# dwave-examples/image-generation

Hardware: AMD Instinct MI355X
Metric: DVAE+GRBM train-step images/s (MNIST) at 1/2/4/8 MI355X; loss parity vs CPU (higher is better)
Workload: dtype f32

## Files before the change

image-generation_amd/csrc/conv_plan.cpp:

```cpp
#include "conv_plan.h"

#include <algorithm>

namespace dvg {

PlanOptions plan_options() {
  PlanOptions o;
  o.precision = conv_precision_mode(); o.launch_mode = conv_launch_mode(0, 0);
  for (int i = 0; i < OPT_COUNT; ++i) o.v[i] = opt((Opt)i);
  return o;
}

namespace {
bool wino_mode_ok(const PlanOptions& o, ConvPass pass) { return pass == PASS_WGRAD || o.precision != 1; }

constexpr int WINO_MIN_BLOCKS = 512;

bool enc_wino_wanted(const PlanOptions& o, int64_t M, int Cout, ConvPass pass, bool training) {
  if (o.v[OPT_ENC_WINO] == 0 || !wino_mode_ok(o, pass)) return false;
  if (o.v[OPT_ENC_WINO] >= 1) return true;
  return conv_wino_blocks(M, Cout) >= (training ? WINO_MIN_BLOCKS : 256);
}

bool wino4_bit(const PlanOptions& o, int64_t mask, int bit) { return o.v[OPT_ENC_WINO4] != 0 && ((mask >> bit) & 1); }

bool wino4_block64(const PlanOptions& o, int l, bool dgrad, int64_t M, int Cin, int Cout, int L, int cus) {
  if (!wino4_bit(o, o.v[OPT_ENC_WINO4_MASK], enc_wino4_block64_bit(l, dgrad)) || !conv_wino4_block64_shape(M, Cin, Cout, L)) return false;
  return (int64_t)conv_wino4_stats_blocks(M) * (Cout / 64) >= 2 * (int64_t)(cus > 0 && cus < 256 ? cus : 256);
}

bool is_wino(ConvForm f) { return f == CF_WINO2 || f == CF_WINO4; }
WeightMap map9(const ConvLayer& y, bool dgrad) {
  const int mode = y.convt ? (dgrad ? WM_CONVT_DGRAD : WM_CONVT_FWD) : (dgrad ? WM_CONV_DGRAD : WM_CONV_FWD);
  return dgrad ? WeightMap{mode, y.Cout, y.Cin, 9} : WeightMap{mode, y.Cin, y.Cout, 9};
}
}

bool plan_enc_wino_fwd(int64_t M, int Cin, int Cout, int L, bool training, const PlanOptions& o) {
  return conv_wino_shape(M, Cin, Cout, L) && enc_wino_wanted(o, M, Cout, PASS_FWD, training);
}

int plan_enc_wino_cus(const PlanOptions& o, ConvPass pass, bool training) {
  if (pass == PASS_FWD) return (training && o.v[OPT_WINO_DYNAMIC] == 0) ? 192 : 0;
  if (pass == PASS_DGRAD) return o.v[OPT_ENC_DGRAD_CUS] > 0 ? (int)o.v[OPT_ENC_DGRAD_CUS] : WINO_CUS_ENC_DGRAD;
  return (int)o.v[OPT_ENC_WGRAD_CUS];
}

void plan_encoder_layers(int64_t B, int n, bool training, const PlanOptions& o, ConvLayer y[4]) {
  const int ch[5] = {1, 32, 64, 128, n};
  for (int l = 1; l < 4; ++l) {
    ConvLayer& c = y[l];
    c.M = B * (1024 >> (2 * l)); c.Cin = ch[l]; c.Cout = ch[l + 1]; c.L = 5 - l; c.ups = false; c.convt = false;
    c.form[PASS_FWD] = c.form[PASS_DGRAD] = c.form[PASS_WGRAD] = CF_DIRECT;
    c.block64[PASS_FWD] = c.block64[PASS_DGRAD] = false;
    if (plan_enc_wino_fwd(c.M, c.Cin, c.Cout, c.L, training, o))
      c.form[PASS_FWD] = wino4_bit(o, o.v[OPT_ENC_WINO4_MASK], l - 1) && conv_wino4_shape(c.M, c.Cin, c.Cout, c.L) ? CF_WINO4 : CF_WINO2;
    c.block64[PASS_FWD] = c.form[PASS_FWD] == CF_WINO4 &&
                          wino4_block64(o, l, false, c.M, c.Cin, c.Cout, c.L, plan_enc_wino_cus(o, PASS_FWD, training));
    if (!training) continue;
    if (conv_wino_shape(c.M, c.Cout, c.Cin, c.L) && enc_wino_wanted(o, c.M, c.Cin, PASS_DGRAD, true))
      c.form[PASS_DGRAD] = wino4_bit(o, o.v[OPT_ENC_WINO4_MASK], 2 + l) && conv_wino4_shape(c.M, c.Cout, c.Cin, c.L) ? CF_WINO4 : CF_WINO2;
    c.block64[PASS_DGRAD] = c.form[PASS_DGRAD] == CF_WINO4 &&
                            wino4_block64(o, l, true, c.M, c.Cout, c.Cin, c.L, plan_enc_wino_cus(o, PASS_DGRAD, true));
    if (conv_wino_wgrad_shape(c.M, c.Cin, c.Cout, c.L) && enc_wino_wanted(o, c.M, c.Cout, PASS_WGRAD, true) &&
        (o.v[OPT_ENC_WINO] >= 1 || conv_wino_shape(c.M, c.Cin, c.Cout, c.L)))
      c.form[PASS_WGRAD] = wino4_bit(o, o.v[OPT_ENC_WINO4_MASK], 5 + l) && conv_wino4_wgrad_shape(c.M, c.Cin, c.Cout, c.L) ? CF_WINO4 : CF_WINO2;
  }
}

void plan_decoder_layers(int64_t N, int n, const PlanOptions& o, ConvLayer y[3]) {
  const int ch[4] = {n, 128, 64, 32};
  for (int l = 0; l < 3; ++l) {
    ConvLayer& c = y[l];
    c.M = N * ((int64_t)4 << (2 * l)); c.Cin = ch[l]; c.Cout = ch[l + 1]; c.L = l + 1; c.ups = l > 0; c.convt = true;
    c.block64[PASS_FWD] = c.block64[PASS_DGRAD] = false;
    ConvForm base = CF_DIRECT;
    if (l == 0 && o.v[OPT_DEC_D22] != 0)
      base = o.v[OPT_DEC_LC0] != 0 && (o.v[OPT_DEC_LC0] > 0 || N >= 4096 || N * (int64_t)n >= (1 << 20)) && conv_pack_is_f32_kmajor(o.launch_mode) ? CF_LC0 : CF_D22;
    if (c.ups && o.v[OPT_DEC_FOLD] != 0 && conv_fold_ok(c.M / 4)) base = CF_FOLD;
    c.form[PASS_FWD] = c.form[PASS_DGRAD] = c.form[PASS_WGRAD] = base;
    if (!c.ups || o.v[OPT_DEC_WINO] == 0 || (o.v[OPT_DEC_WINO] < 0 && N < 8192)) continue;
// ... 109 lines not shown
```

image-generation_amd/csrc/conv_wino_wgrad.hip:

```cpp
#include <atomic>
#include <type_traits>

#include "conv_wino_common.h"

namespace dvg {

struct WinoWgradArgs {
  const float* in;
  const float* dy;
  float* slabs;
  int64_t M;
  int Cin, Cout, L;
  int isplit;
};

template <int WA, int WB>
struct WinoWgrad8Cfg {
  static constexpr int WK = 4 / (WA * WB);
  static constexpr int CIB = 32 * WA, COB = 32 * WB;
  static constexpr int QC = WK == 1 ? 8 : 4;
  static constexpr int NQ = QC * WK;
  static constexpr int V_B = NQ * CIB * 64, Z_B = NQ * COB * 64, STAGE = V_B + Z_B;
  static constexpr int LDS_BYTES = 2 * STAGE;
  static constexpr int NV = NQ * CIB / 2, NZ = NQ * COB / 2;
// ... 211 lines not shown
        for (int i = 0; i < NM; ++i) {
          if (i % MPG == 0) __builtin_amdgcn_sched_group_barrier(0x100, 2, 0);
          __builtin_amdgcn_sched_group_barrier(0x008, 1, 0);
          if (VPM > 0) __builtin_amdgcn_sched_group_barrier(0x002, VPM, 0);
          if (NST > 0 && ((i + 1) * NST) / NM - (i * NST) / NM >= 1) __builtin_amdgcn_sched_group_barrier(0x200, 1, 0);
          if (NST > 0 && ((i + 1) * NST) / NM - (i * NST) / NM >= 2) __builtin_amdgcn_sched_group_barrier(0x200, 1, 0);
          if (NST > 0 && ((i + 1) * NST) / NM - (i * NST) / NM >= 3) __builtin_amdgcn_sched_group_barrier(0x200, 1, 0);
        }
      }
      __builtin_amdgcn_sched_barrier(0);
#pragma unroll
      for (int e = NH; e < NGRP; ++e) {
        const int g = G0 + e * GSTEP;
        if (e + 1 < NGRP) load_grp(g + GSTEP, na, nb);
#pragma unroll
        for (int m = 0; m < 4; ++m)
          if (!UPS || m != 2)
            acc[4 * (g & 1) + m] = __builtin_amdgcn_mfma_f32_32x32x2f32(ca[m], cb[m], acc[4 * (g & 1) + m], 0, 0, 0);
        ca = na; cb = nb;
        __builtin_amdgcn_sched_group_barrier(0x100, 2, 0);
        __builtin_amdgcn_sched_group_barrier(0x008, MPG, 0);
      }
      __builtin_amdgcn_sched_barrier(0);
      __syncthreads();
    };
    for (int ch = 0; ch < nchunks; ch += 2) {
      chunk(ch, std::integral_constant<int, 0>{});
      chunk(ch + 1, std::integral_constant<int, 1>{});
    }
  };
  using R0 = std::integral_constant<int, 0>;
  using R1 = std::integral_constant<int, 1>;
  using R2 = std::integral_constant<int, 2>;
  using PX = std::integral_constant<int, -1>;
  if constexpr (UPS) {
    if (ps == 0) { if (is_v) run(R0{}, R0{}); else if (is_z) run(R1{}, R0{}); else run(R2{}, R0{}); }
    else { if (is_v) run(R0{}, R1{}); else if (is_z) run(R1{}, R1{}); else run(R2{}, R1{}); }
  } else {
    if (is_v) run(R0{}, PX{}); else if (is_z) run(R1{}, PX{}); else run(R2{}, PX{});
  }

  const size_t slab = ((size_t)blockIdx.z * C::WK + kg) * 16 * (size_t)a.Cin * a.Cout;
#pragma unroll
  for (int j = 0; j < 8; ++j) {
    if (UPS && (j & 3) == 2) continue;
    const int p = 8 * ps + j;
    if (UPS && (p >> 2) == 2) continue;
    float* dst = a.slabs + slab + ((size_t)p * a.Cin + a0 + wa * 32) * a.Cout + b0 + wb * 32 + c;
#pragma unroll
    for (int r = 0; r < 16; ++r) dst[(size_t)crow16(r, hh) * a.Cout] = acc[j][r];
  }
}

__global__ __launch_bounds__(256) void wino_wgrad_slabsum_kernel(float* __restrict__ slabs, int nslabs, int64_t pairs, int positions, int ups) {
  const int64_t total = positions * pairs;
  const int sub = threadIdx.x & 7;
  for (int64_t e = ((int64_t)blockIdx.x * 256 + threadIdx.x) >> 3; e < total; e += ((int64_t)gridDim.x * 256) >> 3) {
    if (ups) {
      const int p = (int)(e / pairs);
      if ((p >> 2) == 2 || (p & 3) == 2) continue;
    }
    float s = 0.f;
    for (int k0 = sub; k0 < nslabs; k0 += 64) {
      float v[8];
#pragma unroll
      for (int u = 0; u < 8; ++u) v[u] = k0 + 8 * u < nslabs ? slabs[(size_t)(k0 + 8 * u) * total + e] : 0.f;
#pragma unroll
      for (int u = 0; u < 8; ++u) if (k0 + 8 * u < nslabs) s += v[u];
    }
    s += __shfl_xor(s, 1, 64);
    s += __shfl_xor(s, 2, 64);
    s += __shfl_xor(s, 4, 64);
    if (sub == 0) slabs[e] = s;
  }
}

int launch_wino_wgrad_slabsum(float* slabs, int nslabs, int64_t pairs, int positions, int ups, hipStream_t s) {
  int64_t blocks = (positions * pairs * 8 + 255) / 256;
  if (blocks > 4096) blocks = 4096;
  DVG_LAUNCH(K_WGRAD_REDUCE, wino_wgrad_slabsum_kernel, dim3((unsigned)blocks), dim3(256), 0, s, slabs, nslabs, pairs, positions, ups);
  return DVG_OK;
}

__global__ __launch_bounds__(256) void wino_wgrad_reduce_kernel(const float* __restrict__ du, WeightMap map, float* __restrict__ grad_w, int ups) {
  const int64_t pairs = (int64_t)map.Ca * map.Cb;
  for (int64_t e = (int64_t)blockIdx.x * 256 + threadIdx.x; e < pairs; e += (int64_t)gridDim.x * 256) {
    float u[16];
#pragma unroll
    for (int p = 0; p < 16; ++p) u[p] = (ups && ((p >> 2) == 2 || (p & 3) == 2)) ? 0.f : du[(size_t)p * pairs + e];
    float t[3][4];
#pragma unroll
    for (int nu = 0; nu < 4; ++nu) {
      t[0][nu] = u[0 * 4 + nu] + 0.5f * (u[1 * 4 + nu] + u[2 * 4 + nu]);
      t[1][nu] = 0.5f * (u[1 * 4 + nu] - u[2 * 4 + nu]);
      t[2][nu] = 0.5f * (u[1 * 4 + nu] + u[2 * 4 + nu]) + u[3 * 4 + nu];
    }
    const int b = (int)(e % map.Cb), av = (int)(e / map.Cb);
#pragma unroll
    for (int r = 0; r < 3; ++r) {
      const float g0 = t[r][0] + 0.5f * (t[r][1] + t[r][2]);
      const float g1 = 0.5f * (t[r][1] - t[r][2]);
      const float g2 = 0.5f * (t[r][1] + t[r][2]) + t[r][3];
      grad_w[torch_weight_offset(map, 3 * r + 0, av, b)] = g0;
      grad_w[torch_weight_offset(map, 3 * r + 1, av, b)] = g1;
      grad_w[torch_weight_offset(map, 3 * r + 2, av, b)] = g2;
    }
  }
}

static bool wino_wgrad_shape_ok(int64_t M, int Cin, int Cout, int L) {
  if (L < 1 || L > 5 || M <= 0 || (M & (((int64_t)1 << (2 * L)) - 1))) return false;
  const bool t22 = Cin % 64 == 0 && Cout % 64 == 0, t12 = Cin == 32 && Cout % 64 == 0, t21 = Cin % 64 == 0 && Cout == 32;
  if (!(t22 || t12 || t21)) return false;
  if (M * (int64_t)(Cin > Cout ? Cin : Cout) * 4 >= 2147483647LL) return false;
  return true;
}
bool conv_wino_wgrad_shape(int64_t M, int Cin, int Cout, int L) { return wino_wgrad_shape_ok(M, Cin, Cout, L); }

struct WinoWgradGeom { int tiles, pgn, isplit, wk, nslabs; };
static WinoWgradGeom wino_wgrad_geom(int64_t M, int Cin, int Cout, int L, int cus) {
  WinoWgradGeom g;
  const bool full = Cin % 64 == 0 && Cout % 64 == 0;
  const int cib = Cin % 64 == 0 ? 64 : 32, cob = Cout % 64 == 0 ? 64 : 32, nq = 8;
  g.wk = full ? 1 : 2;
  g.tiles = (Cin / cib) * (Cout / cob);
  const int qi = 1 << (2 * L - 2);
  g.pgn = qi >= nq ? qi / nq : 1;
  const int ipc = qi >= nq ? 1 : nq / qi;
  const int n_img = (int)(M >> (2 * L));
  const int ichunks = (n_img + ipc - 1) / ipc;
  g.isplit = wino_slab_split(ichunks, g.tiles * g.pgn, cus).want;
  g.nslabs = g.pgn * g.isplit * g.wk;
  return g;
// ... 47 lines not shown
```

image-generation_amd/csrc/dev_hooks.cpp:

```cpp
#include "conv_plan.h"
#include "gibbs_plan.h"
#include "mmd_plan.h"
#include "../../include/dvg_dev.h"
using namespace dvg;

extern "C" int dvg_dev_conv_igemm(const float* in, const float* w, int mode, float* wp, const float* bias, float* out,
                                  float* stats, int64_t M, int Cin, int Cout, int L, int ntaps, int ups, int poolsum,
                                  int repack, float* splitk_ws, dvg_stream_t stream) {
  DVG_REQUIRE(in && w && wp && out, "dev_conv_igemm: null argument");
  hipStream_t s = (hipStream_t)stream;
  if (repack) DVG_TRY(launch_weight_pack(w, WeightMap{mode, Cin, Cout, ntaps}, wp, s, conv_launch_mode(M, Cout)));
  ConvArgs a;
  a.in = in; a.wp = wp; a.bias = bias; a.out = out; a.stats = stats;
  a.M = M; a.Cin = Cin; a.Cout = Cout; a.L = L; a.ntaps = ntaps; a.ups = ups; a.poolsum = poolsum;
  a.splitk_ws = splitk_ws;
  a.spin_a = opt(OPT_DEV_SPIN_OPERAND) != 0;
  return launch_conv_igemm(a, s);
}

extern "C" int dvg_dev_conv_wino(const float* in, const float* w, int mode, float* u, const float* bias, float* out,
                                 float* stats, int64_t M, int Cin, int Cout, int L, dvg_stream_t stream) {
  DVG_REQUIRE(in && w && u && out, "dev_conv_wino: null argument");
  hipStream_t s = (hipStream_t)stream;
  DVG_TRY(launch_wino_weight_pack(w, WeightMap{mode, Cin, Cout, 9}, u, s));
  ConvArgs a;
  a.in = in; a.wp = u; a.bias = bias; a.out = out; a.stats = stats;
  a.M = M; a.Cin = Cin; a.Cout = Cout; a.L = L; a.ntaps = 9; a.ups = 0; a.poolsum = 0;
  a.splitk_ws = nullptr;
  return launch_conv_wino(a, s);
}
extern "C" int dvg_dev_conv_wino4(const float* in, const float* w, int mode, float* u, const float* bias, float* out,
                                  float* stats, int64_t M, int Cin, int Cout, int L, int cus, int um, dvg_stream_t stream) {
  DVG_REQUIRE(in && w && u && out, "dev_conv_wino4: null argument");
  hipStream_t s = (hipStream_t)stream;
  DVG_TRY(launch_wino4_weight_pack(w, WeightMap{mode, Cin, Cout, 9}, u, s, um != 0));
  ConvArgs a;
  a.in = in; a.wp = u; a.bias = bias; a.out = out; a.stats = stats;
  a.M = M; a.Cin = Cin; a.Cout = Cout; a.L = L; a.ntaps = 9; a.ups = 0; a.poolsum = 0;
  a.splitk_ws = nullptr; a.wino_cus = cus; a.wino_um = um;
  const int64_t mask = opt(OPT_ENC_WINO4_MASK);
  a.wino4_block64 = um == 0 && L >= 2 && L <= 4 && ((mask >> enc_wino4_block64_bit(5 - L, mode != 0)) & 1) && conv_wino4_block64_shape(M, Cin, Cout, L);
  return launch_conv_wino4(a, s);
}
extern "C" int dvg_dev_conv_wino4_shape(int64_t M, int Cin, int Cout, int L) { return conv_wino4_shape(M, Cin, Cout, L) ? 1 : 0; }
extern "C" int dvg_dev_conv_wino_ok(int64_t M, int Cin, int Cout, int L) { return plan_enc_wino_fwd(M, Cin, Cout, L, true, plan_options()) ? 1 : 0; }

extern "C" int dvg_dev_plan_forms(int network, int64_t rows, int n_latents, int training, int out[15]) {
  DVG_REQUIRE(out && (network == 0 || network == 1) && rows >= 1 && n_latents >= 32 && n_latents % 32 == 0, "dev_plan_forms: bad argument");
  const PlanOptions o = plan_options();
  ConvLayer y[4];
  if (network == 0) plan_encoder_layers(rows, n_latents, training != 0, o, y);
  else plan_decoder_layers(rows, n_latents, o, y);
  for (int l = 0; l < 4; ++l)
// ... 26 lines not shown
  const int64_t v[19] = {p.form, p.lpc, p.waves, p.mb, p.nr, p.maxs, p.ch, p.fix, p.slots.n, p.chains_per_block, p.grid, p.threads,
                         (int64_t)p.lds, g.lane_has, g.lane_lpc, g.lane_mb, g.lane_nr, g.lane_rows, g.n_batches};
  for (int i = 0; i < 19; ++i) out[i] = v[i];
  return DVG_OK;
}
extern "C" int dvg_dev_gibbs_exchange_plan(int n, int n_colours, const int32_t* class_ptr, const int32_t* adj_ptr, int n_ladders,
                                           int n_replicas, int64_t out[20]) {
  DVG_REQUIRE(out && class_ptr && adj_ptr && n > 0 && n_colours > 0 && n_colours <= 64 && n_ladders > 0 && n_replicas >= 2 &&
                  n_replicas <= GIBBS_MAX_REPLICAS && (int64_t)n_ladders * n_replicas <= 0x7fffffff,
              "dev_gibbs_exchange_plan: bad argument");
  const GibbsGraphShape g = gibbs_graph_shape(n, n_colours, class_ptr, adj_ptr);
  GibbsDrawPlan p;
  int per_block = 0;
  DVG_TRY(gibbs_exchange_plan(g, n_ladders, n_replicas, opt(OPT_GIBBS_GENERIC), &p, &per_block));
  const int64_t v[20] = {p.form, p.lpc, p.waves, p.mb, p.nr, p.maxs, p.ch, p.fix, p.slots.n, p.chains_per_block, p.grid, p.threads,
                         (int64_t)p.lds, g.lane_has, g.lane_lpc, g.lane_mb, g.lane_nr, g.lane_rows, g.n_batches, per_block};
  for (int i = 0; i < 20; ++i) out[i] = v[i];
  return DVG_OK;
}
extern "C" int dvg_dev_conv_wino_stats_blocks(int64_t M, int Cout) { return conv_wino_stats_blocks(M, Cout); }

extern "C" size_t dvg_dev_conv_splitk_floats(int64_t M, int Cin, int Cout, int ntaps, int poolsum) {
  return conv_splitk_floats(M, Cin, Cout, ntaps, poolsum);
}

extern "C" int dvg_dev_conv_stats_blocks(int64_t M, int Cout) { return conv_stats_blocks(M, Cout); }

extern "C" size_t dvg_dev_wgrad_slab_floats(int64_t M, int Cin, int Cout, int ntaps) {
  return (size_t)wgrad_ksplit(M, Cin, Cout, ntaps) * ntaps * Cin * Cout;
}

extern "C" int dvg_dev_conv_wgrad(const float* in, const float* dy, float* slabs, float* grad_w, int mode, int64_t M,
                                  int Cin, int Cout, int L, int ntaps, int ups, dvg_stream_t stream) {
  DVG_REQUIRE(in && dy && slabs && grad_w, "dev_conv_wgrad: null argument");
  hipStream_t s = (hipStream_t)stream;
  WgradArgs wa;
  wa.in = in; wa.dy = dy; wa.slabs = slabs; wa.M = M; wa.Cin = Cin; wa.Cout = Cout; wa.L = L; wa.ntaps = ntaps;
  wa.ups = ups; wa.ksplit = wgrad_ksplit(M, Cin, Cout, ntaps);
  wa.spin_x = opt(OPT_DEV_SPIN_OPERAND) != 0;
  DVG_TRY(launch_conv_wgrad(wa, s));
  return launch_wgrad_reduce(slabs, wa.ksplit, WeightMap{mode, Cin, Cout, ntaps}, grad_w, s);
}

extern "C" size_t dvg_dev_wino_wgrad_slab_floats(int64_t M, int Cin, int Cout, int L) {
  return conv_wino_wgrad_shape(M, Cin, Cout, L) ? conv_wino_wgrad_slab_floats(M, Cin, Cout, L) : 0;
}

extern "C" int dvg_dev_conv_wino_wgrad(const float* in, const float* dy, float* slabs, float* grad_w, int mode, int64_t M,
                                       int Cin, int Cout, int L, int ups, int cus, dvg_stream_t stream) {
  DVG_REQUIRE(in && dy && slabs && grad_w, "dev_conv_wino_wgrad: null argument");
  return launch_conv_wino_wgrad(in, dy, M, Cin, Cout, L, slabs, WeightMap{mode, Cin, Cout, 9}, grad_w, (hipStream_t)stream, ups, cus);
}

extern "C" size_t dvg_dev_wino4_wgrad_slab_floats(int64_t M, int Cin, int Cout, int L) {
  return conv_wino4_wgrad_shape(M, Cin, Cout, L) ? conv_wino4_wgrad_slab_floats(M, Cin, Cout) : 0;
}

extern "C" int dvg_dev_conv_wino4_wgrad(const float* in, const float* dy, float* slabs, float* grad_w, int mode, int64_t M,
                                        int Cin, int Cout, int L, int cus, dvg_stream_t stream) {
  DVG_REQUIRE(in && dy && slabs && grad_w, "dev_conv_wino4_wgrad: null argument");
  return launch_conv_wino4_wgrad(in, dy, M, Cin, Cout, L, slabs, WeightMap{mode, Cin, Cout, 9}, grad_w, (hipStream_t)stream, cus);
}
```

image-generation_amd/csrc/options.cpp:

```cpp
#include <atomic>
#include <cstring>
#include <mutex>

#include "common.h"

namespace dvg {
namespace {
struct OptDef { const char* name; int64_t def; const char* doc; bool dev = false; };
const OptDef kDefs[OPT_COUNT] = {
    {"igemm_dma", 1, "float32 forward / data-gradient GEMM: 1 LDS-DMA staging (default), 0 register staging (tensors of 4 GiB and more always; A/B reference)", true},
    {"igemm_posmajor", 1, "position-major tiles (padding taps of small images never multiplied): 1 on, 0 pixel-major tiles"},
    {"igemm_thr128", 512, "blocks a launch must have for the 128x128 tile (the tests lower it to send small fixtures through that tile)", true},
    {"wgrad_dma", 1, "weight-gradient GEMMs: 1 LDS-DMA staging (default), 0 register staging (tensors of 4 GiB and more always)", true},
    {"dec_fold", 1, "decoder: Upsample(x2) + ConvTranspose as 4 class GEMMs with pre-summed taps (4/9 of the FLOPs)"},
    {"dec_d22", 1, "decoder: first ConvTranspose layer on 2x2 images as one dense map per image (16/36 of the FLOPs)"},
    {"dec_lc0", -1, "decoder: Linear composed with that map: -1 from 4096 rows up or rows x n_latents >= 2^20 (default), 0 never, 1 always"},
    {"mmd_w128", -1, "MMD: 128-row-block pair kernel: -1 by problem size (default), 0 never, 1 whenever the shape allows", true},
    {"mmd_d256", -1, "MMD: 256-row distance-sum kernel: -1 by problem size (default), 0 never, 1 whenever the shape allows", true},
    {"gibbs_generic", 0, "sampler: 1 forces the plain rolled reference schedule (no chains-side-by-side form for large graphs), 2 the lane-major schedule one row at a time instead of two passes of a class side by side, 3 the lane-major schedule whatever the size, 4 the chains-side-by-side schedule in 8-chain workgroups whatever the size (all bit-identical; A/B references)", true},
    {"side_stream", 1, "weight-gradient chains on the library's side stream (0 serialises everything on the caller's)"},
    {"enc_wino", -1, "encoder 3x3 layers in the Winograd F(2x2,3x3) form, forward, data gradient and weight gradient: -1 by size (default: evaluation-mode forward launches of 256 workgroups' worth of tiles or more, training launches of 512 or more), 0 never, 1 every launch the shape allows; forward / data gradient never in the bf16-input mode"},
    {"dec_wino", -1, "decoder Upsample(x2) + 3x3 layers in the Winograd form (9 of 16 transform positions), forward, data gradient and weight gradient: -1 from 8192 decoder rows up (default), 0 never, 1 whenever the shape allows"},
    {"enc_l0_fused", 1, "encoder layer 0: 1 = its output is recomputed by every pass that needs it (BatchNorm statistics, BN/pool/LeakyReLU, the backward sums, the weight gradient) and never stored (default), 0 = stored and re-read (rounds 1-2)", true},
    {"dec_tail_fused", 1, "decoder: 1 = the 8x8x32 stage's BatchNorm / Dropout / LeakyReLU (forward and backward) run inside the 32 -> 1 layer's kernels, its activated map and that map's gradient are never stored (default), 0 = separate passes (rounds 1-2)", true},
    {"wino_dynamic", 1, "Winograd forward / data-gradient launches deal their tile blocks dynamically (an atomic counter per grid row) instead of round-robin: a workgroup that gets its CU late takes fewer blocks (1 default, 0 = the static deal of rounds 3-4)", true},
    {"enc_wino4", 1, "every launch of the Winograd F(4x4,3x3) form -- forward, data gradient and weight gradient, encoder and decoder: 1 (default) the launches that run in the Winograd domain take it where the shape qualifies and their bit of the dev options enc_wino4_mask / dec_wino4_mask is set (36 position GEMMs per 4x4 output tile: 2.25 multiplies per output instead of 4.0; behind the decoder's upsample 25 of the 36), 0 none: the F(2x2,3x3) form everywhere"},
    {"enc_wino4_mask", 0x14013c, "which encoder launches option enc_wino4 covers: bit l-1 the forward of layer l (1..3), bit 2+l its data gradient, bit 5+l its weight gradient (default 0x13c in these bits: layer 3's forward, every data gradient, layer 3's weight gradient -- the forwards of layers 1-2 gain nothing inside the step and their 7x float32 noise in front of two more max-pool stages moved the B = 1024 full-size gradient test from 4.6e-3 to 5.4e-3 of its 5e-3 bar; the weight gradients of layers 1-2 are level with the F(2x2,3x3) kernel); bits 16-21: the BLOCK SHAPE of a forward / data-gradient launch that takes the form -- bit 15+l layer l's forward, bit 18+l its data gradient: set, the launch runs work items of 64 tiles x 64 output channels as two passes of 32 tiles x 64 channels (half the raw-pixel pieces, input transforms and transformed-entry writes per matrix operation, the same bits) where Cout % 64 == 0 and every workgroup of its CU budget gets two items or more; clear, blocks of 64 tiles x 32 channels (the A/B reference); default bits 18 and 20: layer 3's forward and layer 2's data gradient, each measured faster inside the c3 step -- at c3 no other launch of the form qualifies", true},
    {"enc_dgrad_cus", 0, "CUs the encoder's Winograd data-gradient launches are sized for (0: the measured constant of conv.h)", true},
    {"enc_wgrad_cus", 0, "CUs the encoder's Winograd weight-gradient launches are sized for (0: the measured constant of conv.h)", true},
    {"dec_wino4_mask", 0x2, "which of the decoder's Winograd launches behind the upsample take the F(4x4,3x3) form with 25 of 36 positions (option enc_wino4 != 0): bit 0 / 1 the forward of the 128 -> 64 / 64 -> 32 layer (bit 0 off: with it the full-size decoder's reconstruction is 2.97e-6 from float64, the bar is 2e-6), bit 2 / 3 their data gradients", true},
    {"wgrad_reduce_tiled", 1, "weight-gradient slab sums of at most 8 slabs and at least 256 tiles by the tiled one-thread-per-element kernels (same bits; 0: the 8-lanes-per-element kernels everywhere)", true},
    {"enc_bn_reduce_pooled", 1, "encoder BatchNorm/pool backward: the (sum dz, sum dz zhat) pass reads the pooled activations the forward kept (2 floats per element) instead of the four pre-BatchNorm outputs of every window (5); 0: the window form", true},
    {"mmd_gram_fp4", 1, "MMD: exact Gram of +-1 rows on the FP4 matrix pipe (scaled 32x32x64 MFMA on a packed e2m1 copy of the rows: the same integers at half the operand bytes and k-steps) in the 256-row distance-sum kernel and the 128-row-block pair kernel at d = 256, 512 (default); 0: the int8 form (A/B reference, same bits)", true},
    {"dec_spin_gemm", 1, "decoder input layer on spins the caller declared +-1 (dvg_decoder_declare_spins): 1 (default) its forward GEMM and its weight-gradient GEMM multiply the spins as exact bf16 values with the float32 operand as three bf16 pieces (three exact products on the bf16 matrix pipe); 2 the forward GEMM alone (A/B runs); 0 every declaration is ignored: the kernels of the operand mode, bit for bit", true},
    {"dev_spin_operand", 0, "test knob: 1 = the development hooks dvg_dev_conv_igemm / dvg_dev_conv_wgrad make the +-1 promise for their input operand", true},
};
std::atomic<int64_t> g_val[OPT_COUNT];
std::once_flag g_once;
void init_once() {
  std::call_once(g_once, [] {
    for (int i = 0; i < OPT_COUNT; ++i) g_val[i].store(kDefs[i].def, std::memory_order_relaxed);
  });
}
}

int64_t opt(Opt id) {
  init_once();
  return g_val[id].load(std::memory_order_relaxed);
}
}

using namespace dvg;

namespace {
int nth(bool dev, int i) {
  for (int k = 0; k < OPT_COUNT; ++k)
    if (kDefs[k].dev == dev && i-- == 0) return k;
  return -1;
}
int count(bool dev) {
  int n = 0;
  for (int k = 0; k < OPT_COUNT; ++k) n += kDefs[k].dev == dev;
  return n;
}
int set_opt(bool dev, const char* what, const char* name, int64_t value) {
  DVG_REQUIRE(name, "%s: null name", what);
  init_once();
  for (int i = 0; i < OPT_COUNT; ++i)
    if (kDefs[i].dev == dev && !strcmp(name, kDefs[i].name)) { g_val[i].store(value, std::memory_order_relaxed); return DVG_OK; }
  set_error("%s: unknown option '%s'", what, name);
  return DVG_E_INVALID;
}
int get_opt(bool dev, const char* what, const char* name, int64_t* value) {
  DVG_REQUIRE(name && value, "%s: null argument", what);
  init_once();
  for (int i = 0; i < OPT_COUNT; ++i)
    if (kDefs[i].dev == dev && !strcmp(name, kDefs[i].name)) { *value = g_val[i].load(std::memory_order_relaxed); return DVG_OK; }
  set_error("%s: unknown option '%s'", what, name);
  return DVG_E_INVALID;
}
// ... 20 lines not shown
```

image-generation_amd/dev.py:

```python
import ctypes

import numpy as np
import torch

from . import _lib

_SIGS = {
    "dvg_dev_conv_igemm": (ctypes.c_int, [ctypes.c_void_p] * 2 + [ctypes.c_int] + [ctypes.c_void_p] * 4 +
                           [ctypes.c_int64] + [ctypes.c_int] * 7 + [ctypes.c_void_p, ctypes.c_void_p]),
    "dvg_dev_conv_splitk_floats": (ctypes.c_size_t, [ctypes.c_int64, ctypes.c_int, ctypes.c_int, ctypes.c_int, ctypes.c_int]),
    "dvg_dev_conv_stats_blocks": (ctypes.c_int, [ctypes.c_int64, ctypes.c_int]),
    "dvg_dev_conv_wino": (ctypes.c_int, [ctypes.c_void_p] * 2 + [ctypes.c_int] + [ctypes.c_void_p] * 4 +
                          [ctypes.c_int64] + [ctypes.c_int] * 3 + [ctypes.c_void_p]),
    "dvg_dev_conv_wino4": (ctypes.c_int, [ctypes.c_void_p] * 2 + [ctypes.c_int] + [ctypes.c_void_p] * 4 +
                           [ctypes.c_int64] + [ctypes.c_int] * 5 + [ctypes.c_void_p]),
    "dvg_dev_conv_wino4_shape": (ctypes.c_int, [ctypes.c_int64, ctypes.c_int, ctypes.c_int, ctypes.c_int]),
    "dvg_dev_wino4_wgrad_slab_floats": (ctypes.c_size_t, [ctypes.c_int64, ctypes.c_int, ctypes.c_int, ctypes.c_int]),
    "dvg_dev_conv_wino4_wgrad": (ctypes.c_int, [ctypes.c_void_p] * 4 + [ctypes.c_int, ctypes.c_int64] + [ctypes.c_int] * 4 +
                                 [ctypes.c_void_p]),
    "dvg_dev_conv_wino_ok": (ctypes.c_int, [ctypes.c_int64, ctypes.c_int, ctypes.c_int, ctypes.c_int]),
    "dvg_dev_plan_forms": (ctypes.c_int, [ctypes.c_int, ctypes.c_int64, ctypes.c_int, ctypes.c_int, ctypes.POINTER(ctypes.c_int)]),
    "dvg_dev_mmd_plan": (ctypes.c_int, [ctypes.c_int64, ctypes.c_int64, ctypes.c_int, ctypes.POINTER(ctypes.c_int64)]),
    "dvg_dev_gibbs_draw_plan": (ctypes.c_int, [ctypes.c_int, ctypes.c_int, ctypes.c_void_p, ctypes.c_void_p, ctypes.c_int, ctypes.c_int,
                                               ctypes.POINTER(ctypes.c_int64)]),
    "dvg_dev_gibbs_exchange_plan": (ctypes.c_int, [ctypes.c_int, ctypes.c_int, ctypes.c_void_p, ctypes.c_void_p, ctypes.c_int, ctypes.c_int,
                                                   ctypes.POINTER(ctypes.c_int64)]),
    "dvg_dev_conv_wino_stats_blocks": (ctypes.c_int, [ctypes.c_int64, ctypes.c_int]),
    "dvg_dev_wgrad_slab_floats": (ctypes.c_size_t, [ctypes.c_int64, ctypes.c_int, ctypes.c_int, ctypes.c_int]),
    "dvg_dev_conv_wgrad": (ctypes.c_int, [ctypes.c_void_p] * 4 + [ctypes.c_int, ctypes.c_int64] + [ctypes.c_int] * 5 +
                           [ctypes.c_void_p]),
    "dvg_dev_encoder_layout": (ctypes.c_int, [ctypes.c_int64, ctypes.c_int, ctypes.POINTER(ctypes.c_size_t)]),
    "dvg_dev_wino_wgrad_slab_floats": (ctypes.c_size_t, [ctypes.c_int64, ctypes.c_int, ctypes.c_int, ctypes.c_int]),
    "dvg_dev_conv_wino_wgrad": (ctypes.c_int, [ctypes.c_void_p] * 4 + [ctypes.c_int, ctypes.c_int64] + [ctypes.c_int] * 5 +
                                [ctypes.c_void_p]),
}
_bound = False


def lib():
    global _bound
    L = _lib.lib()
    if not _bound:
        for name, (res, args) in _SIGS.items():
            fn = getattr(L, name)
            fn.restype, fn.argtypes = res, args
        _bound = True
    return L


def morton_perm(side: int) -> torch.Tensor:
    def compact(v):
        v &= 0x55555555
        v = (v | (v >> 1)) & 0x33333333
        v = (v | (v >> 2)) & 0x0F0F0F0F
        v = (v | (v >> 4)) & 0x00FF00FF
        return v
    m = np.arange(side * side)
    return torch.from_numpy((compact(m >> 1) * side + compact(m)).astype(np.int64))


def nchw_to_morton(x: torch.Tensor) -> torch.Tensor:
    N, C, H, W = x.shape
    perm = morton_perm(H).to(x.device)
    return x.permute(0, 2, 3, 1).reshape(N, H * W, C)[:, perm, :].reshape(N * H * W, C).contiguous()


def morton_to_nchw(t: torch.Tensor, N: int, C: int, side: int) -> torch.Tensor:
    perm = morton_perm(side).to(t.device)
    out = torch.empty((N, side * side, C), dtype=t.dtype, device=t.device)
    out[:, perm, :] = t.reshape(N, side * side, C)
    return out.reshape(N, side, side, C).permute(0, 3, 1, 2).contiguous()


def conv_igemm(x_m, w, mode, M, Cin, Cout, L, ntaps=9, ups=0, poolsum=0, bias=None, stats=False, wp=None, repack=True,
               splitk=True):
    Lb = lib()
    dev = x_m.device
    wp = wp if wp is not None else torch.empty((ntaps * Cin * Cout * 3 + 1) // 2, device=dev)
    out = torch.empty(((M // 4) if poolsum else M, Cout), device=dev)
    st = torch.empty((Lb.dvg_dev_conv_stats_blocks(M, Cout), Cout, 2), device=dev) if stats else None
    nsk = Lb.dvg_dev_conv_splitk_floats(M, Cin, Cout, ntaps, poolsum) if splitk else 0
    sk = torch.empty(nsk, device=dev) if nsk else None
    _lib.check(Lb.dvg_dev_conv_igemm(x_m.data_ptr(), w.data_ptr(), mode, wp.data_ptr(), _lib.ptr(bias), out.data_ptr(),
                                     _lib.ptr(st), M, Cin, Cout, L, ntaps, ups, poolsum, int(repack), _lib.ptr(sk),
                                     _lib.stream_ptr(dev)))
    return (out, st) if stats else out

# ... 58 lines not shown
    o = (ctypes.c_int64 * 20)()
    _lib.check(lib().dvg_dev_gibbs_exchange_plan(int(plan.n), int(plan.n_colours), class_ptr.ctypes.data, adj_ptr.ctypes.data,
                                                 int(n_ladders), int(n_replicas), o), "dvg_dev_gibbs_exchange_plan")
    return dict(_gibbs_plan_dict(o), ladders_per_workgroup=o[19])


def conv_wino(x_m, w, mode, M, Cin, Cout, L, bias=None, stats=False):
    Lb = lib()
    dev = x_m.device
    u = torch.empty(16 * Cin * Cout, device=dev)
    out = torch.empty((M, Cout), device=dev)
    st = torch.empty((Lb.dvg_dev_conv_wino_stats_blocks(M, Cout), Cout, 2), device=dev) if stats else None
    _lib.check(Lb.dvg_dev_conv_wino(x_m.data_ptr(), w.data_ptr(), mode, u.data_ptr(), _lib.ptr(bias), out.data_ptr(),
                                    _lib.ptr(st), M, Cin, Cout, L, _lib.stream_ptr(dev)))
    return (out, st) if stats else out


def conv_wino4_shape(M, Cin, Cout, L):
    return bool(lib().dvg_dev_conv_wino4_shape(M, Cin, Cout, L))


def conv_wino4(x_m, w, mode, M, Cin, Cout, L, bias=None, stats=False, cus=0, um=0):
    Lb = lib()
    dev = x_m.device
    u = torch.empty(36 * Cin * Cout, device=dev)
    out = torch.empty((M // 4 if um == 2 else M, Cout), device=dev)
    st = torch.empty((M // 1024, Cout, 2), device=dev) if stats else None
    _lib.check(Lb.dvg_dev_conv_wino4(x_m.data_ptr(), w.data_ptr(), mode, u.data_ptr(), _lib.ptr(bias), out.data_ptr(),
                                     _lib.ptr(st), M, Cin, Cout, L, int(cus), int(um), _lib.stream_ptr(dev)))
    return (out, st) if stats else out


def conv_wgrad(x_m, dy, mode, w_shape, M, Cin, Cout, L, ntaps=9, ups=0):
    Lb = lib()
    dev = x_m.device
    slabs = torch.empty(Lb.dvg_dev_wgrad_slab_floats(M, Cin, Cout, ntaps), device=dev)
    gw = torch.empty(w_shape, device=dev)
    _lib.check(Lb.dvg_dev_conv_wgrad(x_m.data_ptr(), dy.data_ptr(), slabs.data_ptr(), gw.data_ptr(), mode, M, Cin, Cout, L,
                                     ntaps, ups, _lib.stream_ptr(dev)))
    return gw


def conv_wino_wgrad(x_m, dy, mode, w_shape, M, Cin, Cout, L, ups=0, cus=0):
    Lb = lib()
    dev = x_m.device
    nf = Lb.dvg_dev_wino_wgrad_slab_floats(M, Cin, Cout, L)
    if nf == 0:
        return None
    slabs = torch.empty(nf, device=dev)
    gw = torch.empty(w_shape, device=dev)
    _lib.check(Lb.dvg_dev_conv_wino_wgrad(x_m.data_ptr(), dy.data_ptr(), slabs.data_ptr(), gw.data_ptr(), mode, M, Cin, Cout, L,
                                          int(ups), int(cus), _lib.stream_ptr(dev)))
    return gw


def encoder_saved(ws: torch.Tensor, B: int, n: int):
    off = (ctypes.c_size_t * 16)()
    _lib.check(lib().dvg_dev_encoder_layout(B, n, off), "dvg_dev_encoder_layout")
    f = ws.view(torch.float32)
    ch = [32, 64, 128, n]
    out = []
    for l in range(4):
        side, C = 32 >> l, ch[l]
        y = f[off[l]: off[l] + B * side * side * C]
        stored = l > 0 or _lib.get_option("enc_l0_fused") == 0
        out.append(dict(Y=morton_to_nchw(y, B, C, side) if stored else None, mean=f[off[8 + l]: off[8 + l] + C], invstd=f[off[12 + l]: off[12 + l] + C]))
    return out


def conv_wino4_wgrad(x_m, dy, mode, w_shape, M, Cin, Cout, L, cus=0):
    Lb = lib()
    dev = x_m.device
    nf = Lb.dvg_dev_wino4_wgrad_slab_floats(M, Cin, Cout, L)
    if nf == 0:
        return None
    slabs = torch.empty(nf, device=dev)
    gw = torch.empty(w_shape, device=dev)
    _lib.check(Lb.dvg_dev_conv_wino4_wgrad(x_m.data_ptr(), dy.data_ptr(), slabs.data_ptr(), gw.data_ptr(), mode, M, Cin, Cout, L,
                                           int(cus), _lib.stream_ptr(dev)))
    return gw
```

include/dvg_dev.h:

```cpp
#ifndef DVG_DEV_H
#define DVG_DEV_H
#include "dvg.h"
#ifdef __cplusplus
extern "C" {
#endif
int dvg_dev_conv_igemm(const float *in, const float *w, int mode, float *wp, const float *bias, float *out,
                       float *stats, int64_t M, int Cin, int Cout, int L, int ntaps, int ups, int poolsum,
                       int repack, float *splitk_ws, dvg_stream_t stream);
size_t dvg_dev_conv_splitk_floats(int64_t M, int Cin, int Cout, int ntaps, int poolsum);
int dvg_dev_conv_wino(const float *in, const float *w, int mode, float *u, const float *bias, float *out, float *stats,
                      int64_t M, int Cin, int Cout, int L, dvg_stream_t stream);
int dvg_dev_conv_wino_ok(int64_t M, int Cin, int Cout, int L);
int dvg_dev_plan_forms(int network, int64_t rows, int n_latents, int training, int out[15]);
int dvg_dev_mmd_plan(int64_t nx, int64_t ny, int dim, int64_t out[24]);
int dvg_dev_gibbs_draw_plan(int n, int n_colours, const int32_t *class_ptr, const int32_t *adj_ptr, int n_chains, int kind,
                            int64_t out[19]);
int dvg_dev_gibbs_exchange_plan(int n, int n_colours, const int32_t *class_ptr, const int32_t *adj_ptr, int n_ladders,
                                int n_replicas, int64_t out[20]);
int dvg_dev_conv_wino4(const float *in, const float *w, int mode, float *u, const float *bias, float *out, float *stats,
                       int64_t M, int Cin, int Cout, int L, int cus, int um, dvg_stream_t stream);
int dvg_dev_conv_wino4_shape(int64_t M, int Cin, int Cout, int L);
size_t dvg_dev_wino4_wgrad_slab_floats(int64_t M, int Cin, int Cout, int L);
int dvg_dev_conv_wino4_wgrad(const float *in, const float *dy, float *slabs, float *grad_w, int mode, int64_t M, int Cin,
                             int Cout, int L, int cus, dvg_stream_t stream);
int dvg_dev_conv_wino_stats_blocks(int64_t M, int Cout);
int dvg_dev_conv_stats_blocks(int64_t M, int Cout);
size_t dvg_dev_wgrad_slab_floats(int64_t M, int Cin, int Cout, int ntaps);
int dvg_dev_conv_wgrad(const float *in, const float *dy, float *slabs, float *grad_w, int mode, int64_t M, int Cin,
                       int Cout, int L, int ntaps, int ups, dvg_stream_t stream);
size_t dvg_dev_wino_wgrad_slab_floats(int64_t M, int Cin, int Cout, int L);
int dvg_dev_conv_wino_wgrad(const float *in, const float *dy, float *slabs, float *grad_w, int mode, int64_t M, int Cin,
                            int Cout, int L, int ups, int cus, dvg_stream_t stream);
int dvg_dev_encoder_layout(int64_t B, int n_latents, size_t out[16]);
int dvg_dev_option_count(void);
const char *dvg_dev_option_name(int index);
const char *dvg_dev_option_doc(int index);
int dvg_dev_set_option(const char *name, int64_t value);
int dvg_dev_get_option(const char *name, int64_t *value);
#ifdef __cplusplus
}
#endif
#endif
```

Baseline: 607,700.

## Vectorize Winograd weight-gradient slab sum and widen 64x64 block-shape eligibility

The slab reduction kernel now has each thread read float4 vectors from up to 16 slabs, splitting slabs across 1-8 thread groups that combine partials through shared memory, instead of 8 lanes summing scalars and shuffling. The goal is fewer, wider loads that stream the slab buffer at higher bandwidth. The 64-tile x 64-channel block shape is now also chosen when the work items divide evenly across the workgroups, and the default mask turns it on for layer 3's data gradient. New asserts limit the slabsum to pairs divisible by 4 and 16 or 36 positions, and a test hook for the slabsum kernel is exposed.

Result: no change. 613,100 (median of 6 runs) (+0.9%).

```diff
diff --git a/image-generation_amd/csrc/conv_plan.cpp b/image-generation_amd/csrc/conv_plan.cpp
--- a/image-generation_amd/csrc/conv_plan.cpp
+++ b/image-generation_amd/csrc/conv_plan.cpp
@@ -26,7 +26,8 @@
 
 bool wino4_block64(const PlanOptions& o, int l, bool dgrad, int64_t M, int Cin, int Cout, int L, int cus) {
   if (!wino4_bit(o, o.v[OPT_ENC_WINO4_MASK], enc_wino4_block64_bit(l, dgrad)) || !conv_wino4_block64_shape(M, Cin, Cout, L)) return false;
-  return (int64_t)conv_wino4_stats_blocks(M) * (Cout / 64) >= 2 * (int64_t)(cus > 0 && cus < 256 ? cus : 256);
+  const int64_t items = (int64_t)conv_wino4_stats_blocks(M) * (Cout / 64), wgs = cus > 0 && cus < 256 ? cus : 256;
+  return items >= 2 * wgs || (items >= wgs && items % wgs == 0);
 }
 
 bool is_wino(ConvForm f) { return f == CF_WINO2 || f == CF_WINO4; }
diff --git a/image-generation_amd/csrc/conv_wino_wgrad.hip b/image-generation_amd/csrc/conv_wino_wgrad.hip
--- a/image-generation_amd/csrc/conv_wino_wgrad.hip
+++ b/image-generation_amd/csrc/conv_wino_wgrad.hip
@@ -287,33 +287,47 @@
   }
 }
 
-__global__ __launch_bounds__(256) void wino_wgrad_slabsum_kernel(float* __restrict__ slabs, int nslabs, int64_t pairs, int positions, int ups) {
+__global__ __launch_bounds__(256) void wino_wgrad_slabsum_kernel(float* __restrict__ slabs, int nslabs, int64_t pairs, int positions, int ups, int csh) {
+  constexpr int NF = 16;
+  __shared__ f32x4 part[256];
   const int64_t total = positions * pairs;
-  const int sub = threadIdx.x & 7;
-  for (int64_t e = ((int64_t)blockIdx.x * 256 + threadIdx.x) >> 3; e < total; e += ((int64_t)gridDim.x * 256) >> 3) {
-    if (ups) {
-      const int p = (int)(e / pairs);
-      if ((p >> 2) == 2 || (p & 3) == 2) continue;
-    }
-    float s = 0.f;
-    for (int k0 = sub; k0 < nslabs; k0 += 64) {
-      float v[8];
-#pragma unroll
-      for (int u = 0; u < 8; ++u) v[u] = k0 + 8 * u < nslabs ? slabs[(size_t)(k0 + 8 * u) * total + e] : 0.f;
-#pragma unroll
-      for (int u = 0; u < 8; ++u) if (k0 + 8 * u < nslabs) s += v[u];
-    }
-    s += __shfl_xor(s, 1, 64);
-    s += __shfl_xor(s, 2, 64);
-    s += __shfl_xor(s, 4, 64);
-    if (sub == 0) slabs[e] = s;
-  }
+  const int cols = 256 >> csh, col = (int)threadIdx.x & (cols - 1), c = (int)threadIdx.x >> (8 - csh);
+  const int64_t e = ((int64_t)blockIdx.x * cols + col) * 4;
+  bool live = e < total;
+  if (live && ups) {
+    const int p = (int)(e / pairs);
+    live = !((p >> 2) == 2 || (p & 3) == 2);
+  }
+  f32x4 s = {0.f, 0.f, 0.f, 0.f};
+  if (live) {
+    const float* src = slabs + e;
+    for (int k0 = c; k0 < nslabs; k0 += 8 * NF) {
+      f32x4 v[NF];
+#pragma unroll
+      for (int u = 0; u < NF; ++u)
+        if (k0 + 8 * u < nslabs) v[u] = *reinterpret_cast<const f32x4*>(src + (size_t)(k0 + 8 * u) * total);
+#pragma unroll
+      for (int u = 0; u < NF; ++u)
+        if (k0 + 8 * u < nslabs) s += v[u];
+    }
+  }
+  part[threadIdx.x] = s;
+  __syncthreads();
+  if (c != 0 || !live) return;
+  f32x4 q[8];
+#pragma unroll
+  for (int i = 0; i < 8; ++i) q[i] = i < (1 << csh) ? part[i * cols + col] : (f32x4){0.f, 0.f, 0.f, 0.f};
+  *reinterpret_cast<f32x4*>(slabs + e) = ((q[0] + q[1]) + (q[2] + q[3])) + ((q[4] + q[5]) + (q[6] + q[7]));
 }
 
 int launch_wino_wgrad_slabsum(float* slabs, int nslabs, int64_t pairs, int positions, int ups, hipStream_t s) {
-  int64_t blocks = (positions * pairs * 8 + 255) / 256;
-  if (blocks > 4096) blocks = 4096;
-  DVG_LAUNCH(K_WGRAD_REDUCE, wino_wgrad_slabsum_kernel, dim3((unsigned)blocks), dim3(256), 0, s, slabs, nslabs, pairs, positions, ups);
+  DVG_REQUIRE(slabs && nslabs >= 1 && pairs >= 4 && pairs % 4 == 0 && (positions == 16 || (positions == 36 && !ups)),
+              "wino_wgrad_slabsum: unsupported launch (nslabs=%d pairs=%lld positions=%d ups=%d)", nslabs, (long long)pairs, positions, ups);
+  int csh = 0;
+  while (csh < 3 && (1 << csh) < nslabs) ++csh;
+  const int64_t cols = 256 >> csh, blocks = (positions * pairs / 4 + cols - 1) / cols;
+  DVG_REQUIRE(blocks <= 0x7fffffff, "wino_wgrad_slabsum: too many elements (pairs=%lld)", (long long)pairs);
+  DVG_LAUNCH(K_WGRAD_REDUCE, wino_wgrad_slabsum_kernel, dim3((unsigned)blocks), dim3(256), 0, s, slabs, nslabs, pairs, positions, ups, csh);
   return DVG_OK;
 }
 
diff --git a/image-generation_amd/csrc/dev_hooks.cpp b/image-generation_amd/csrc/dev_hooks.cpp
--- a/image-generation_amd/csrc/dev_hooks.cpp
+++ b/image-generation_amd/csrc/dev_hooks.cpp
@@ -1,4 +1,5 @@
 #include "conv_plan.h"
+#include "conv_wino_common.h"
 #include "gibbs_plan.h"
 #include "mmd_plan.h"
 #include "../../include/dvg_dev.h"
@@ -131,6 +132,11 @@
   return launch_conv_wino_wgrad(in, dy, M, Cin, Cout, L, slabs, WeightMap{mode, Cin, Cout, 9}, grad_w, (hipStream_t)stream, ups, cus);
 }
 
+extern "C" int dvg_dev_wino_slabsum(float* slabs, int nslabs, int64_t pairs, int positions, int ups, dvg_stream_t stream) {
+  DVG_REQUIRE(slabs, "dev_wino_slabsum: null argument");
+  return launch_wino_wgrad_slabsum(slabs, nslabs, pairs, positions, ups, (hipStream_t)stream);
+}
+
 extern "C" size_t dvg_dev_wino4_wgrad_slab_floats(int64_t M, int Cin, int Cout, int L) {
   return conv_wino4_wgrad_shape(M, Cin, Cout, L) ? conv_wino4_wgrad_slab_floats(M, Cin, Cout) : 0;
 }
diff --git a/image-generation_amd/csrc/options.cpp b/image-generation_amd/csrc/options.cpp
--- a/image-generation_amd/csrc/options.cpp
+++ b/image-generation_amd/csrc/options.cpp
@@ -25,7 +25,7 @@
     {"dec_tail_fused", 1, "decoder: 1 = the 8x8x32 stage's BatchNorm / Dropout / LeakyReLU (forward and backward) run inside the 32 -> 1 layer's kernels, its activated map and that map's gradient are never stored (default), 0 = separate passes (rounds 1-2)", true},
     {"wino_dynamic", 1, "Winograd forward / data-gradient launches deal their tile blocks dynamically (an atomic counter per grid row) instead of round-robin: a workgroup that gets its CU late takes fewer blocks (1 default, 0 = the static deal of rounds 3-4)", true},
     {"enc_wino4", 1, "every launch of the Winograd F(4x4,3x3) form -- forward, data gradient and weight gradient, encoder and decoder: 1 (default) the launches that run in the Winograd domain take it where the shape qualifies and their bit of the dev options enc_wino4_mask / dec_wino4_mask is set (36 position GEMMs per 4x4 output tile: 2.25 multiplies per output instead of 4.0; behind the decoder's upsample 25 of the 36), 0 none: the F(2x2,3x3) form everywhere"},
-    {"enc_wino4_mask", 0x14013c, "which encoder launches option enc_wino4 covers: bit l-1 the forward of layer l (1..3), bit 2+l its data gradient, bit 5+l its weight gradient (default 0x13c in these bits: layer 3's forward, every data gradient, layer 3's weight gradient -- the forwards of layers 1-2 gain nothing inside the step and their 7x float32 noise in front of two more max-pool stages moved the B = 1024 full-size gradient test from 4.6e-3 to 5.4e-3 of its 5e-3 bar; the weight gradients of layers 1-2 are level with the F(2x2,3x3) kernel); bits 16-21: the BLOCK SHAPE of a forward / data-gradient launch that takes the form -- bit 15+l layer l's forward, bit 18+l its data gradient: set, the launch runs work items of 64 tiles x 64 output channels as two passes of 32 tiles x 64 channels (half the raw-pixel pieces, input transforms and transformed-entry writes per matrix operation, the same bits) where Cout % 64 == 0 and every workgroup of its CU budget gets two items or more; clear, blocks of 64 tiles x 32 channels (the A/B reference); default bits 18 and 20: layer 3's forward and layer 2's data gradient, each measured faster inside the c3 step -- at c3 no other launch of the form qualifies", true},
+    {"enc_wino4_mask", 0x34013c, "which encoder launches option enc_wino4 covers: bit l-1 the forward of layer l (1..3), bit 2+l its data gradient, bit 5+l its weight gradient (default 0x13c in these bits: layer 3's forward, every data gradient, layer 3's weight gradient -- the forwards of layers 1-2 gain nothing inside the step and their 7x float32 noise in front of two more max-pool stages moved the B = 1024 full-size gradient test from 4.6e-3 to 5.4e-3 of its 5e-3 bar; the weight gradients of layers 1-2 are level with the F(2x2,3x3) kernel); bits 16-21: the BLOCK SHAPE of a forward / data-gradient launch that takes the form -- bit 15+l layer l's forward, bit 18+l its data gradient: set, the launch runs work items of 64 tiles x 64 output channels as two passes of 32 tiles x 64 channels (half the raw-pixel pieces, input transforms and transformed-entry writes per matrix operation, the same bits) where Cout % 64 == 0 and every workgroup of its CU budget gets two items or more, or a whole number of them (at least one); clear, blocks of 64 tiles x 32 channels (the A/B reference); default bits 18, 20 and 21: layer 3's forward and the data gradients of layers 2 and 3, each measured faster inside the c3 step (layer 3's data gradient there: 128 items on its 128 CUs) -- at c3 no other launch of the form qualifies", true},
     {"enc_dgrad_cus", 0, "CUs the encoder's Winograd data-gradient launches are sized for (0: the measured constant of conv.h)", true},
     {"enc_wgrad_cus", 0, "CUs the encoder's Winograd weight-gradient launches are sized for (0: the measured constant of conv.h)", true},
     {"dec_wino4_mask", 0x2, "which of the decoder's Winograd launches behind the upsample take the F(4x4,3x3) form with 25 of 36 positions (option enc_wino4 != 0): bit 0 / 1 the forward of the 128 -> 64 / 64 -> 32 layer (bit 0 off: with it the full-size decoder's reconstruction is 2.97e-6 from float64, the bar is 2e-6), bit 2 / 3 their data gradients", true},
diff --git a/image-generation_amd/dev.py b/image-generation_amd/dev.py
--- a/image-generation_amd/dev.py
+++ b/image-generation_amd/dev.py
@@ -33,6 +33,8 @@
     "dvg_dev_wino_wgrad_slab_floats": (ctypes.c_size_t, [ctypes.c_int64, ctypes.c_int, ctypes.c_int, ctypes.c_int]),
     "dvg_dev_conv_wino_wgrad": (ctypes.c_int, [ctypes.c_void_p] * 4 + [ctypes.c_int, ctypes.c_int64] + [ctypes.c_int] * 5 +
                                 [ctypes.c_void_p]),
+    "dvg_dev_wino_slabsum": (ctypes.c_int, [ctypes.c_void_p, ctypes.c_int, ctypes.c_int64, ctypes.c_int, ctypes.c_int,
+                                            ctypes.c_void_p]),
 }
 _bound = False
 
@@ -197,6 +199,13 @@
     _lib.check(Lb.dvg_dev_conv_wino_wgrad(x_m.data_ptr(), dy.data_ptr(), slabs.data_ptr(), gw.data_ptr(), mode, M, Cin, Cout, L,
                                           int(ups), int(cus), _lib.stream_ptr(dev)))
     return gw
+
+
+def wino_slabsum(slabs, nslabs, pairs, positions, ups):
+    assert slabs.dtype == torch.float32 and slabs.is_contiguous() and slabs.numel() >= nslabs * positions * pairs
+    _lib.check(lib().dvg_dev_wino_slabsum(slabs.data_ptr(), int(nslabs), int(pairs), int(positions), int(ups),
+                                          _lib.stream_ptr(slabs.device)))
+    return slabs.view(-1)[: positions * pairs].view(positions, pairs)
 
 
 def encoder_saved(ws: torch.Tensor, B: int, n: int):
diff --git a/include/dvg_dev.h b/include/dvg_dev.h
--- a/include/dvg_dev.h
+++ b/include/dvg_dev.h
@@ -31,6 +31,7 @@
 size_t dvg_dev_wino_wgrad_slab_floats(int64_t M, int Cin, int Cout, int L);
 int dvg_dev_conv_wino_wgrad(const float *in, const float *dy, float *slabs, float *grad_w, int mode, int64_t M, int Cin,
                             int Cout, int L, int ups, int cus, dvg_stream_t stream);
+int dvg_dev_wino_slabsum(float *slabs, int nslabs, int64_t pairs, int positions, int ups, dvg_stream_t stream);
 int dvg_dev_encoder_layout(int64_t B, int n_latents, size_t out[16]);
 int dvg_dev_option_count(void);
 const char *dvg_dev_option_name(int index);
```
